# lucidrains/DALLE-pytorch

Hardware: AMD Instinct MI355X
Metric: img-tokens/sec (higher is better)
Workload: dtype bf16; 1 GPU; model=dalle-dim1024-depth12-heads16, reversible=True, global_batch=64, seq_len=1280, image_seq_len=1024, parallelism=dp1, mode=train, eager=False

## Files before the change

### dalle_pytorch_amd/models/reversible.py

```python

import torch
import torch.nn as nn
from torch.autograd.function import Function
from torch.utils.checkpoint import get_device_states, set_device_states


def route_args(router, args, depth):
    routed = [({}, {}) for _ in range(depth)]
    for key, per_layer in router.items():
        if key not in args:
            continue
        val = args[key]
        for i, (f_on, g_on) in enumerate(per_layer):
            if f_on:
                routed[i][0][key] = val
            if g_on:
                routed[i][1][key] = val
    return routed


class Deterministic(nn.Module):

    def __init__(self, net):
        super().__init__()
        self.net = net
        self._cpu_state = None
        self._gpu_devices = None
        self._gpu_states = None
        self._had_gpu = False
        self._autocast = None

    def record_rng(self, *tensors):
        self._cpu_state = torch.get_rng_state()
        if torch.cuda._initialized:
            self._had_gpu = True
            self._gpu_devices, self._gpu_states = get_device_states(*tensors)
        self._autocast = (torch.is_autocast_enabled('cuda'),
                          torch.get_autocast_dtype('cuda'))

    def forward(self, *args, record_rng=False, set_rng=False, **kwargs):
        if record_rng:
            self.record_rng(*args)
        if not set_rng:
            return self.net(*args, **kwargs)
        devices = self._gpu_devices if self._had_gpu else []
        with torch.random.fork_rng(devices=devices, enabled=True):
            torch.set_rng_state(self._cpu_state)
            if self._had_gpu:
                set_device_states(self._gpu_devices, self._gpu_states)
            if self._autocast is not None and self._autocast[0] and torch.cuda.is_available():
                with torch.autocast('cuda', dtype=self._autocast[1], enabled=True):
                    return self.net(*args, **kwargs)
            return self.net(*args, **kwargs)


def _residual_branch(det, inp, residual, record_rng, args):
    if getattr(det.net, 'supports_residual', False):
        return det(inp, residual=residual, record_rng=record_rng, **args)
    return residual + det(inp, record_rng=record_rng, **args)


class ReversibleBlock(nn.Module):

    def __init__(self, f, g):
        super().__init__()
        self.f = Deterministic(f)
        self.g = Deterministic(g)

    def forward(self, x1, x2, f_args={}, g_args={}):
        rec = self.training
        with torch.no_grad():
            y1 = _residual_branch(self.f, x2, x1, rec, f_args)
            y2 = _residual_branch(self.g, y1, x2, rec, g_args)
        return y1, y2

    @staticmethod
    def _replay_grad(det, inp, upstream, args):
        leaf = inp.detach().requires_grad_(True)
        with torch.enable_grad():
            out = det(leaf, set_rng=True, **args)
        torch.autograd.backward(out, upstream)
        return out.detach(), leaf.grad

    def backward_pass(self, y1, y2, dy1, dy2, f_args={}, g_args={}):
        gy1, dy1_via_g = self._replay_grad(self.g, y1, dy2, g_args)
        x2 = y2 - gy1
        dx1 = dy1 + dy1_via_g
        del y2, gy1, dy1, dy1_via_g
        fx2, dx2_via_f = self._replay_grad(self.f, x2, dx1, f_args)
        x1 = y1 - fx2
        dx2 = dy2 + dx2_via_f
        del y1, fx2, dy2, dx2_via_f
        return x1, x2, dx1, dx2


class _ReversibleFunction(Function):
    @staticmethod
    def forward(ctx, x1, x2, blocks, args):
        ctx.args = args
        for block, kw in zip(blocks, args):
            x1, x2 = block(x1, x2, **kw)
        ctx.y1 = x1.detach()
        ctx.y2 = x2.detach()
        ctx.blocks = blocks
        return x1, x2

    @staticmethod
    def backward(ctx, dy1, dy2):
        y1, y2 = ctx.y1, ctx.y2
        for block, kw in zip(ctx.blocks[::-1], ctx.args[::-1]):
            y1, y2, dy1, dy2 = block.backward_pass(y1, y2, dy1, dy2, **kw)
        return dy1, dy2, None, None


class SequentialSequence(nn.Module):
# ... 31 lines not shown
```

### dalle_pytorch_amd/models/transformer.py

```python

from collections import deque
from collections.abc import Iterable
from functools import partial
from itertools import islice, cycle

import torch
import torch.nn.functional as F
from torch import nn

from dalle_pytorch_amd.models.reversible import ReversibleSequence, SequentialSequence
from dalle_pytorch_amd.models.attention import (
    Attention, SparseAttention, SparseConvCausalAttention, SparseAxialCausalAttention)
from dalle_pytorch_amd.models.positional import build_dalle_rotary_table
from dalle_pytorch_amd.ops import geglu
from dalle_pytorch_amd.ops.fp8 import fp8_linear
from dalle_pytorch_amd.ops.fused import (token_shift, token_shift_supported,
                                          layer_norm, add_scaled)


def _as_tuple(val, depth=1):
    return val if isinstance(val, Iterable) else (val,) * depth


class DivideMax(nn.Module):

    def __init__(self, dim):
        super().__init__()
        self.dim = dim

    def forward(self, x):
        maxes = x.amax(dim=self.dim, keepdim=True).detach()
        return x / maxes


class NonCached(nn.Module):

    def __init__(self, fn):
        super().__init__()
        self.fn = fn

# ... 26 lines not shown

    def __init__(self, dim, depth, fn):
        super().__init__()
        init_eps = next(eps for bound, eps in self.INIT_BY_DEPTH
                        if depth <= bound)
        self.scale = nn.Parameter(torch.full((1, 1, dim), init_eps))
        self.fn = fn

    def forward(self, x, residual=None, **kwargs):
        out = self.fn(x, **kwargs)
        if residual is not None:
            return add_scaled(residual, out, self.scale)
        return out * self.scale.to(out.dtype)


class PreNorm(nn.Module):

    def __init__(self, dim, fn, sandwich=False):
        super().__init__()
        self.norm = nn.LayerNorm(dim)
        self.norm_out = nn.LayerNorm(dim) if sandwich else nn.Identity()
        self.fn = fn

    def forward(self, x, **kwargs):
        y = layer_norm(x, self.norm.weight, self.norm.bias, self.norm.eps)
        y = self.fn(y, **kwargs)
        if isinstance(self.norm_out, nn.LayerNorm):
            y = layer_norm(y, self.norm_out.weight, self.norm_out.bias,
                           self.norm_out.eps)
        return y


class GEGLU(nn.Module):
    def forward(self, x):
        return geglu(x)


class FeedForward(nn.Module):

    def __init__(self, dim, dropout=0., mult=4.):
        super().__init__()
        self.net = nn.Sequential(
            nn.Linear(dim, int(dim * mult * 2)),
            GEGLU(),
            nn.Dropout(dropout),
            nn.Linear(int(dim * mult), dim),
        )

    def forward(self, x, cache=None, cache_key=None):
        x = fp8_linear(self.net[0], x)
        x = self.net[2](self.net[1](x))
        return fp8_linear(self.net[3], x)


class PreShiftToken(nn.Module):

    def __init__(self, fn, image_size, seq_len):
        super().__init__()
        self.fn = fn
        self.image_size = image_size
        self.seq_len = seq_len
        self.img_seq_len = image_size ** 2
        self.text_len = seq_len - self.img_seq_len + 1

    def _shift_full(self, x):
        b, n, c = x.shape
        t, S, q = self.text_len, self.image_size, x.shape[-1] // 4
        prev = x[:, :t - 1, :c // 2]
        text = torch.cat((
            torch.cat((x.new_zeros(b, 1, c // 2), prev), dim=1),
            x[:, :t, c // 2:]), dim=-1)
        img = x[:, t:]
        ni = img.shape[1]
        if ni == 0:
# ... 174 lines not shown
```

### dalle_pytorch_amd/ops/fp8.py

```python

import os
import weakref

import torch
import torch.nn.functional as F

from dalle_pytorch_amd.ops.dispatch import hip_module, using_eager_fallback

_FORCED = None
FP8_MAX = 448.0


def set_fp8_enabled(flag):
    global _FORCED
    _FORCED = bool(flag) if flag is not None else None


def fp8_enabled():
    if _FORCED is not None:
        return _FORCED
    return os.environ.get('DALLE_AMD_FP8', '0') == '1'


_w_cache = {}
_generation = 0


def _owner(w):
    base = w._base
    return base if base is not None else w
# ... 121 lines not shown
    return n * 2 >= k * 3


def _fast_dgrad_ok(x, w):
    if using_eager_fallback(x) or x.dtype != torch.bfloat16:
        return False
    rows = x.numel() // x.shape[-1]
    return (rows >= 1024 and rows % 16 == 0 and w.shape[0] % 16 == 0
            and w.shape[1] % 16 == 0 and torch.is_grad_enabled())


def fp8_linear(linear_module, x):
    w = linear_module.weight
    if _fp8_ok(x, w):
        bias = linear_module.bias
        if bias is not None and bias.dtype != torch.bfloat16:
            bias = bias.to(torch.bfloat16)
        return _Fp8LinearFn.apply(x.contiguous(), w, bias)
    if _fast_dgrad_ok(x, w):
        return _FastDgradLinearFn.apply(x.contiguous(), w, linear_module.bias)
    return linear_module(x)


def fp8_linear_raw(x, weight, bias):
    if _fp8_ok(x, weight) and weight.is_contiguous():
        if bias is not None and bias.dtype != torch.bfloat16:
            bias = bias.to(torch.bfloat16)
        return _Fp8LinearFn.apply(x.contiguous(), weight, bias)
    if _fast_dgrad_ok(x, weight) and weight.is_contiguous():
        return _FastDgradLinearFn.apply(x.contiguous(), weight, bias)
    return F.linear(x, weight, bias)
```

### dalle_pytorch_amd/ops/fused.py

```python

import torch
import torch.nn.functional as F

from dalle_pytorch_amd.ops.dispatch import hip_module, using_eager_fallback


class _GegluFn(torch.autograd.Function):
    @staticmethod
    def forward(ctx, x):
        ext = hip_module()
        x = x.contiguous()
        out = ext.geglu_fwd(x)
        ctx.save_for_backward(x)
        return out

    @staticmethod
    def backward(ctx, dout):
        ext = hip_module()
        (x,) = ctx.saved_tensors
        return ext.geglu_bwd(x, dout.contiguous())


def geglu(x: torch.Tensor) -> torch.Tensor:
    if using_eager_fallback(x) or x.shape[-1] % 16:
# ... 35 lines not shown
        out = ext.resls_fwd(x.contiguous(), y, gf)
        ctx.save_for_backward(y, gf)
        ctx.gamma_meta = (gamma.shape, gamma.dtype)
        return out

    @staticmethod
    def backward(ctx, dout):
        ext = hip_module()
        y, gf = ctx.saved_tensors
        dout = dout.contiguous()
        dy, dgamma = ext.resls_bwd(dout, y, gf)
        shape, dtype = ctx.gamma_meta
        return dout, dy, dgamma.reshape(shape).to(dtype)


def add_scaled(x, y, gamma):
    if (x.is_cuda and x.dtype == torch.bfloat16 and y.dtype == torch.bfloat16
            and not using_eager_fallback(x) and x.shape[-1] % 8 == 0
            and x.shape[-1] // 8 <= 256 and 256 % (x.shape[-1] // 8) == 0):
        return _AddScaledFn.apply(x, y, gamma)
    return x + y * gamma.to(y.dtype)


class _LayerNormFn(torch.autograd.Function):
    @staticmethod
    def forward(ctx, x, weight, bias, eps):
        ext = hip_module()
        y, mean, rstd = ext.ln_fwd(x.contiguous(), weight, bias, eps)
        ctx.save_for_backward(x, weight, mean, rstd)
        return y

    @staticmethod
    def backward(ctx, dy):
        ext = hip_module()
        x, weight, mean, rstd = ctx.saved_tensors
        dx, dgamma, dbeta = ext.ln_bwd(x, dy.contiguous(), weight, mean, rstd)
        return dx, dgamma.to(weight.dtype), dbeta.to(weight.dtype), None


_LN_DIMS = (512, 1024, 1536, 2048)


def layer_norm(x, weight, bias, eps=1e-5):
    if (x.is_cuda and x.dtype == torch.bfloat16 and x.shape[-1] in _LN_DIMS
            and not using_eager_fallback(x)):
        return _LayerNormFn.apply(x, weight, bias, eps)
    if weight is not None and weight.dtype != x.dtype and x.dtype != torch.float32:
        weight = weight.to(x.dtype)
        bias = bias.to(x.dtype) if bias is not None else None
    return F.layer_norm(x, (x.shape[-1],), weight, bias, eps)
```

### dalle_pytorch_amd/ops/hip/hip_ops.hip

```cpp

#include <torch/extension.h>
#include <ATen/hip/HIPContext.h>
#include <hip/hip_runtime.h>

#define DEVFN __device__ __forceinline__

using bf16x8 = __attribute__((ext_vector_type(8))) short;
using bf16x4 = __attribute__((ext_vector_type(4))) short;
using f32x4 = __attribute__((ext_vector_type(4))) float;
using int4v = __attribute__((ext_vector_type(4))) int;

constexpr float NEG_INF = -INFINITY;

DEVFN float bf2f(short u) {
  union { unsigned int i; float f; } c;
  c.i = (unsigned int)(unsigned short)u << 16;
  return c.f;
}
DEVFN short f2bf(float f) {
  union { unsigned int i; float f; } c;
  c.f = f;
  unsigned int r = c.i + 0x7fff + ((c.i >> 16) & 1);
  return (short)(r >> 16);
}
// ... 1621 lines not shown
  #pragma unroll
  for (int e = 0; e < 8; ++e) g[e] = gamma[ch + e];
  for (long r = (long)blockIdx.x * rpp + rg; r < rows;
       r += (long)gridDim.x * rpp) {
    const long base = r * dim + ch;
    int4v dv = *reinterpret_cast<const int4v*>(dout + base);
    int4v yv = *reinterpret_cast<const int4v*>(y + base);
    const short* ds_ = reinterpret_cast<const short*>(&dv);
    const short* ys = reinterpret_cast<const short*>(&yv);
    short o[8];
    #pragma unroll
    for (int e = 0; e < 8; ++e) {
      const float d = bf2f(ds_[e]);
      o[e] = f2bf(g[e] * d);
      dg[e] += d * bf2f(ys[e]);
    }
    *reinterpret_cast<int4v*>(dy + base) = *reinterpret_cast<int4v*>(o);
  }
  const long prow = (long)blockIdx.x * rpp + rg;
  #pragma unroll
  for (int e = 0; e < 8; ++e) dg_part[prow * dim + ch + e] = dg[e];
}


template <int CPT>
__global__ __launch_bounds__(256)
void dec_prelude_kernel(
    const short* __restrict__ x,
    const short* __restrict__ y,
    const float* __restrict__ scale,
    const float* __restrict__ w,
    const float* __restrict__ bia,
    short* __restrict__ xn,
    short* __restrict__ z,
    short* __restrict__ ring,
    const long* __restrict__ offset,
    long rows, float eps, int S, int text_len) {
  constexpr int dim = CPT * 256;
  __shared__ float stat[8];
  const long row = blockIdx.x;
  const int tid = threadIdx.x;
  const int c0 = tid * CPT;
  const short* xr = x + row * (long)dim;
  const short* yr = y ? y + row * (long)dim : nullptr;

  float sum = 0.f, sq = 0.f;
// ... 241 lines not shown
                                      long rows, int H) {
  const long row = blockIdx.y;
  const int i0 = (blockIdx.x * blockDim.x + threadIdx.x) * 8;
  if (row >= rows || i0 >= H) return;
  int4v av = *reinterpret_cast<const int4v*>(x + row * (2L * H) + i0);
  int4v gv = *reinterpret_cast<const int4v*>(x + row * (2L * H) + H + i0);
  int4v dv = *reinterpret_cast<const int4v*>(dout + row * (long)H + i0);
  const short* a = reinterpret_cast<const short*>(&av);
  const short* g = reinterpret_cast<const short*>(&gv);
  const short* d = reinterpret_cast<const short*>(&dv);
  short da[8], dg[8];
  #pragma unroll
  for (int e = 0; e < 8; ++e) {
    const float afv = bf2f(a[e]), gfv = bf2f(g[e]), dfv = bf2f(d[e]);
    da[e] = f2bf(dfv * gelu_f(gfv));
    dg[e] = f2bf(dfv * afv * gelu_grad_f(gfv));
  }
  *reinterpret_cast<int4v*>(dx + row * (2L * H) + i0) =
      *reinterpret_cast<const int4v*>(da);
  *reinterpret_cast<int4v*>(dx + row * (2L * H) + H + i0) =
      *reinterpret_cast<const int4v*>(dg);
}

template <typename T>
__global__ void geglu_fwd_kernel(const T* __restrict__ x, T* __restrict__ out,
                                 long rows, int H) {
  const long row = blockIdx.y;
  const int i0 = (blockIdx.x * blockDim.x + threadIdx.x) * 8;
  if (row >= rows || i0 >= H) return;
  const T* a = x + row * (2L * H) + i0;
  const T* g = a + H;
  T* o = out + row * (long)H + i0;
  #pragma unroll
  for (int e = 0; e < 8; ++e)
    if (i0 + e < H) o[e] = T(float(a[e]) * gelu_f(float(g[e])));
}

template <typename T>
__global__ void geglu_bwd_kernel(const T* __restrict__ x,
                                 const T* __restrict__ dout,
                                 T* __restrict__ dx, long rows, int H) {
  const long row = blockIdx.y;
  const int i0 = (blockIdx.x * blockDim.x + threadIdx.x) * 8;
  if (row >= rows || i0 >= H) return;
  const T* a = x + row * (2L * H) + i0;
  const T* g = a + H;
// ... 473 lines not shown
  const int i = blockIdx.x * blockDim.x + threadIdx.x;
  if (i >= dim) return;
  const long g0 = *offset - text_len;
  const long g = g0 < 0 ? 0 : g0;
  const int pos = (int)(g % S);
  const int prev = (int)(((g - 1) % S + S) % S);
  const int half = dim / 2, quarter = dim / 4;

  short val;
  if (i < quarter) {
    val = ring[((long)bi * S + pos) * half + i];
  } else if (i < half) {
    val = (g % S == 0) ? (short)0
        : ring[((long)bi * S + prev) * half + i];
  } else {
    val = x[(long)bi * dim + i];
  }
  if (i < half) ring[((long)bi * S + pos) * half + i] = x[(long)bi * dim + i];
  out[(long)bi * dim + i] = val;
}



template <int PER>
__global__ __launch_bounds__(256)
void ln_fwd_kernel(const short* __restrict__ x, const float* __restrict__ w,
                   const float* __restrict__ bia, short* __restrict__ y,
                   float* __restrict__ mean_out, float* __restrict__ rstd_out,
                   long rows, float eps) {
  constexpr int per = PER;
  constexpr int dim = PER * 64;
  const long row0 = ((long)blockIdx.x * 4 + (threadIdx.x >> 6)) * 2;
  const int lane = threadIdx.x & 63;
  if (row0 >= rows) return;
  const bool two = row0 + 1 < rows;

  float vals[2][PER];
  #pragma unroll
  for (int rr = 0; rr < 2; ++rr) {
    if (rr && !two) break;
    const short* xr = x + (row0 + rr) * (long)dim;
    #pragma unroll
    for (int i = 0; i < per; i += 8) {
      int4v v = *reinterpret_cast<const int4v*>(xr + lane * per + i);
      const short* vs = reinterpret_cast<const short*>(&v);
      #pragma unroll
      for (int e = 0; e < 8; ++e) vals[rr][i + e] = bf2f(vs[e]);
    }
  }
  #pragma unroll
  for (int rr = 0; rr < 2; ++rr) {
    if (rr && !two) break;
    float sum = 0.f, sq = 0.f;
    #pragma unroll
    for (int i = 0; i < per; ++i) {
      sum += vals[rr][i];
      sq += vals[rr][i] * vals[rr][i];
    }
    #pragma unroll
    for (int sft = 32; sft > 0; sft >>= 1) {
      sum += __shfl_xor(sum, sft);
      sq += __shfl_xor(sq, sft);
    }
    const float mu = sum / dim;
    const float var = sq / dim - mu * mu;
    const float rstd = __frsqrt_rn(var + eps);
    if (lane == 0) {
      mean_out[row0 + rr] = mu;
      rstd_out[row0 + rr] = rstd;
    }
    short* yr = y + (row0 + rr) * (long)dim;
    #pragma unroll
    for (int i = 0; i < per; i += 8) {
      short out8[8];
      #pragma unroll
      for (int e = 0; e < 8; ++e) {
        const int d = lane * per + i + e;
        out8[e] = f2bf((vals[rr][i + e] - mu) * rstd * w[d] + bia[d]);
      }
      *reinterpret_cast<int4v*>(yr + lane * per + i) =
          *reinterpret_cast<const int4v*>(out8);
    }
  }
}

template <int PER>
__global__ __launch_bounds__(256)
void ln_bwd_kernel(const short* __restrict__ x, const short* __restrict__ dy,
                   const float* __restrict__ w,
                   const float* __restrict__ mean_in,
                   const float* __restrict__ rstd_in,
                   short* __restrict__ dx,
                   float* __restrict__ dgamma_part,
                   float* __restrict__ dbeta_part,
                   long rows) {
  constexpr int per = PER;
  constexpr int dim = PER * 64;
  const int block_row0 = blockIdx.x * 4;
  const int wrow = threadIdx.x >> 6;
  const int lane = threadIdx.x & 63;
  const int gridrows = gridDim.x * 4;

  float dgp[PER], dbp[PER];
  #pragma unroll
  for (int i = 0; i < per; ++i) { dgp[i] = 0.f; dbp[i] = 0.f; }

  for (long row = block_row0 + wrow; row < rows; row += gridrows) {
    const short* xr = x + row * dim;
    const short* dyr = dy + row * dim;
    const float mu = mean_in[row];
    const float rstd = rstd_in[row];

    float xh[PER], g[PER];
    float s1 = 0.f, s2 = 0.f;
    #pragma unroll
    for (int i = 0; i < per; i += 8) {
      int4v xv = *reinterpret_cast<const int4v*>(xr + lane * per + i);
      int4v dv = *reinterpret_cast<const int4v*>(dyr + lane * per + i);
      const short* xs = reinterpret_cast<const short*>(&xv);
      const short* ds_ = reinterpret_cast<const short*>(&dv);
      #pragma unroll
      for (int e = 0; e < 8; ++e) {
        const int d = lane * per + i + e;
        const float xhat = (bf2f(xs[e]) - mu) * rstd;
        const float dyv = bf2f(ds_[e]);
        const float gv = dyv * w[d];
        xh[i + e] = xhat;
        g[i + e] = gv;
        s1 += gv;
        s2 += gv * xhat;
        dgp[i + e] += dyv * xhat;
        dbp[i + e] += dyv;
      }
    }
    #pragma unroll
    for (int sft = 32; sft > 0; sft >>= 1) {
      s1 += __shfl_xor(s1, sft);
      s2 += __shfl_xor(s2, sft);
    }
    s1 /= dim;
    s2 /= dim;
    short* dxr = dx + row * (long)dim;
    #pragma unroll
    for (int i = 0; i < per; i += 8) {
      short out8[8];
      #pragma unroll
      for (int e = 0; e < 8; ++e)
        out8[e] = f2bf((g[i + e] - s1 - xh[i + e] * s2) * rstd);
      *reinterpret_cast<int4v*>(dxr + lane * per + i) =
          *reinterpret_cast<const int4v*>(out8);
    }
  }
  float* dgr = dgamma_part + ((long)blockIdx.x * 4 + wrow) * dim;
  float* dbr = dbeta_part + ((long)blockIdx.x * 4 + wrow) * dim;
  #pragma unroll
  for (int i = 0; i < per; ++i) {
    dgr[lane * per + i] = dgp[i];
    dbr[lane * per + i] = dbp[i];
  }
}


__global__ void mfma_probe_kernel(const short* __restrict__ A,
                                  const short* __restrict__ B,
                                  float* __restrict__ C) {
  const int lane = threadIdx.x & 63;
  const int lq = lane & 15, grp = lane >> 4;
  bf16x8 af = *reinterpret_cast<const bf16x8*>(A + lq * 32 + 8 * grp);
  bf16x8 bf;
  #pragma unroll
  for (int e = 0; e < 8; ++e) bf[e] = B[(8 * grp + e) * 16 + lq];
// ... 246 lines not shown
  return out;
}

torch::Tensor geglu_bwd(torch::Tensor x, torch::Tensor dout) {
  CHK(x.is_cuda() && x.is_contiguous() && dout.is_contiguous());
  const int H = (int)x.size(-1) / 2;
  const long rows = x.numel() / (2L * H);
  auto dx = torch::empty_like(x);
  dim3 grid((H + 256 * 8 - 1) / (256 * 8), rows);
  if (x.dtype() == torch::kBFloat16 && H % 8 == 0) {
    hipLaunchKernelGGL(geglu_bwd_bf16_kernel, grid, dim3(256), 0, cur_stream(),
                       reinterpret_cast<const short*>(x.data_ptr()),
                       reinterpret_cast<const short*>(dout.data_ptr()),
                       reinterpret_cast<short*>(dx.data_ptr()), rows, H);
    return dx;
  }
  AT_DISPATCH_FLOATING_TYPES_AND2(at::ScalarType::BFloat16, at::ScalarType::Half,
                                  x.scalar_type(), "geglu_bwd", [&] {
    hipLaunchKernelGGL(geglu_bwd_kernel<scalar_t>, grid, dim3(256), 0, cur_stream(),
                       x.data_ptr<scalar_t>(), dout.data_ptr<scalar_t>(),
                       dx.data_ptr<scalar_t>(), rows, H);
  });
  return dx;
}

torch::Tensor fa_decode(torch::Tensor qkv, torch::Tensor kc, torch::Tensor vc,
                        std::optional<torch::Tensor> cosv,
                        std::optional<torch::Tensor> sinv,
                        torch::Tensor offset,
                        std::optional<torch::Tensor> pattern,
                        double scale,
                        std::optional<torch::Tensor> live,
                        std::optional<torch::Tensor> live_cnt) {
  CHK(qkv.is_cuda() && qkv.dtype() == torch::kBFloat16 && qkv.is_contiguous());
  CHK(kc.is_contiguous() && vc.is_contiguous());
  const int b = kc.size(0), h = kc.size(1), N = kc.size(2);
  CHK(kc.size(3) == 64 && N <= DEC_MAXN);
  CHK(offset.dtype() == torch::kLong);
  int rot = 0;
  const float* cp = nullptr;
  const float* sp = nullptr;
  if (cosv.has_value()) {
    rot = cosv->size(1);
    cp = cosv->data_ptr<float>();
    sp = sinv->data_ptr<float>();
  }
// ... 105 lines not shown
                     C.data_ptr<float>());
  return C;
}


std::vector<torch::Tensor> ln_fwd(torch::Tensor x, torch::Tensor w,
                                  torch::Tensor b, double eps) {
  CHK(x.is_cuda() && x.dtype() == torch::kBFloat16 && x.is_contiguous());
  const int dim = x.size(-1);

  const long rows = x.numel() / dim;
  auto y = torch::empty_like(x);
  auto mean = torch::empty({rows}, x.options().dtype(torch::kFloat32));
  auto rstd = torch::empty_like(mean);
  auto wf = w.to(torch::kFloat32).contiguous();
  auto bf_ = b.to(torch::kFloat32).contiguous();
  dim3 grid((rows + 7) / 8);
  auto launch = [&](auto kern) {
    hipLaunchKernelGGL(kern, grid, dim3(256), 0, cur_stream(),
                       reinterpret_cast<const short*>(x.data_ptr()),
                       wf.data_ptr<float>(), bf_.data_ptr<float>(),
                       reinterpret_cast<short*>(y.data_ptr()),
                       mean.data_ptr<float>(), rstd.data_ptr<float>(),
                       rows, (float)eps);
  };
  switch (dim) {
    case 512: launch(ln_fwd_kernel<8>); break;
    case 1024: launch(ln_fwd_kernel<16>); break;
    case 1536: launch(ln_fwd_kernel<24>); break;
    case 2048: launch(ln_fwd_kernel<32>); break;
    default: TORCH_CHECK(false, "ln_fwd: unsupported dim ", dim);
  }
  return {y, mean, rstd};
}

std::vector<torch::Tensor> ln_bwd(torch::Tensor x, torch::Tensor dy,
                                  torch::Tensor w, torch::Tensor mean,
                                  torch::Tensor rstd) {
  CHK(x.is_cuda() && x.is_contiguous() && dy.is_contiguous());
  const int dim = x.size(-1);
  const long rows = x.numel() / dim;
  auto dx = torch::empty_like(x);
  const long cap = std::min<long>((rows + 3) / 4, 512);
  auto dgp = torch::empty({cap * 4, (long)dim}, x.options().dtype(torch::kFloat32));
  auto dbp = torch::empty_like(dgp);
  auto wf = w.to(torch::kFloat32).contiguous();
  dim3 grid(cap);
  auto launch = [&](auto kern) {
    hipLaunchKernelGGL(kern, grid, dim3(256), 0, cur_stream(),
                       reinterpret_cast<const short*>(x.data_ptr()),
                       reinterpret_cast<const short*>(dy.data_ptr()),
                       wf.data_ptr<float>(), mean.data_ptr<float>(),
                       rstd.data_ptr<float>(),
                       reinterpret_cast<short*>(dx.data_ptr()),
                       dgp.data_ptr<float>(), dbp.data_ptr<float>(), rows);
  };
  switch (dim) {
    case 512: launch(ln_bwd_kernel<8>); break;
    case 1024: launch(ln_bwd_kernel<16>); break;
    case 1536: launch(ln_bwd_kernel<24>); break;
    case 2048: launch(ln_bwd_kernel<32>); break;
    default: TORCH_CHECK(false, "ln_bwd: unsupported dim ", dim);
  }
  auto dgamma = dgp.sum(0);
  auto dbeta = dbp.sum(0);
  return {dx, dgamma, dbeta};
}

std::vector<torch::Tensor> dec_prelude(
    torch::Tensor x, std::optional<torch::Tensor> y,
    std::optional<torch::Tensor> scale,
    torch::Tensor w, torch::Tensor b,
    std::optional<torch::Tensor> ring, torch::Tensor offset,
    double eps, int64_t S, int64_t text_len) {
  CHK(x.is_cuda() && x.dtype() == torch::kBFloat16 && x.is_contiguous());
  CHK(w.dtype() == torch::kFloat32 && b.dtype() == torch::kFloat32);
  const int dim = x.size(-1);
  const long rows = x.numel() / dim;
  const short* yp = nullptr;
  const float* sp_ = nullptr;
  torch::Tensor xn = x;
  if (y.has_value()) {
    CHK(y->is_contiguous() && scale.has_value());
    CHK(scale->dtype() == torch::kFloat32 && scale->is_contiguous());
    yp = reinterpret_cast<const short*>(y->data_ptr());
    sp_ = scale->data_ptr<float>();
    xn = torch::empty_like(x);
  }
  short* rp = nullptr;
// ... 194 lines not shown
                     gamma.data_ptr<float>(),
                     reinterpret_cast<short*>(out.data_ptr()), rows, dim);
  return out;
}

std::vector<torch::Tensor> resls_bwd(torch::Tensor dout, torch::Tensor y,
                                     torch::Tensor gamma) {
  CHK(dout.is_cuda() && dout.dtype() == torch::kBFloat16);
  CHK(dout.is_contiguous() && y.is_contiguous() && gamma.is_contiguous());
  const int dim = dout.size(-1);
  const long rows = dout.numel() / dim;
  auto dy = torch::empty_like(dout);
  const int rpp = 256 / (dim >> 3);
  const long nb = std::min<long>((rows + rpp - 1) / rpp, 1024);
  auto dgp = torch::zeros({nb * rpp, (long)dim},
                          dout.options().dtype(torch::kFloat32));
  hipLaunchKernelGGL(resls_bwd_kernel, dim3(nb), dim3(256), 0, cur_stream(),
                     reinterpret_cast<const short*>(dout.data_ptr()),
                     reinterpret_cast<const short*>(y.data_ptr()),
                     gamma.data_ptr<float>(),
                     reinterpret_cast<short*>(dy.data_ptr()),
                     dgp.data_ptr<float>(), rows, dim);
  return {dy, dgp.sum(0)};
}

PYBIND11_MODULE(TORCH_EXTENSION_NAME, m) {
  m.def("resls_fwd", &resls_fwd, "fused residual + per-channel scale fwd");
  m.def("resls_bwd", &resls_bwd, "fused residual + per-channel scale bwd");
  m.def("quant_fp8", &quant_fp8, "bf16 -> e4m3 one-pass quantize");
  m.def("sample_topk_gumbel", &sample_topk_gumbel,
        py::arg("logits"), py::arg("noise"), py::arg("k"),
        py::arg("temperature"), py::arg("out_tok") = std::nullopt,
        py::arg("seq") = std::nullopt, py::arg("seq_ptr") = std::nullopt,
        "fused top-k threshold + gumbel argmax sampling");
  m.def("amax_bf16", &amax_bf16, "abs-max of a bf16 tensor (one pass)");
  m.def("sk2", &sk2,
        py::arg("x"), py::arg("wp"), py::arg("bias"), py::arg("N"),
        py::arg("K"), py::arg("mode"), py::arg("wscale") = 1.0,
        "decode skinny GEMM on packed bf16/e4m3 weights "
        "(fused bias/geglu/fp32 head)");
  m.def("skinny_gemm", &skinny_gemm,
        "skinny-M weights-streaming GEMM (decode projections)",
        py::arg("x"), py::arg("w"), py::arg("bias") = std::nullopt);
  m.def("dec_prelude", &dec_prelude,
        "fused decode residual + LayerNorm + token-shift");
  m.def("permlane_probe", &permlane_probe,
        "v_permlane32_swap_b32 semantics probe");
  m.def("fa_fwd", &fa_fwd, "flash attention forward (gfx950, d=64)",
        py::arg("q"), py::arg("k"), py::arg("v"), py::arg("scale"),
        py::arg("causal"), py::arg("key_mask"), py::arg("static_mask"),
        py::arg("tile_map"), py::arg("out_bnhd"),
        py::arg("ax_t") = 0, py::arg("ax_S") = 0, py::arg("ax_axis") = -1);
  m.def("fa_bwd", &fa_bwd, "flash attention backward (gfx950, d=64)",
        py::arg("q"), py::arg("k"), py::arg("v"), py::arg("out"),
        py::arg("lse"), py::arg("dout"), py::arg("scale"), py::arg("causal"),
        py::arg("key_mask"), py::arg("static_mask"), py::arg("tile_map"),
        py::arg("tile_map_t"), py::arg("out_bnhd"),
        py::arg("grad_lse") = std::nullopt,
        py::arg("ax_t") = 0, py::arg("ax_S") = 0, py::arg("ax_axis") = -1);
  m.def("rope_split_fwd", &rope_split_fwd,
        "fused qkv split + rotary (q,k,v all rotated)");
  m.def("rope_split_bwd", &rope_split_bwd, "rope_split backward");
  m.def("token_shift", &token_shift, "fused token shift (fwd/transpose)");
  m.def("fa_decode", &fa_decode, "fused single-token decode attention");
  m.def("shift_decode", &shift_decode, "fused single-token token shift");
  m.def("ln_fwd", &ln_fwd, "fused LayerNorm forward (bf16 rows)");
  m.def("ln_bwd", &ln_bwd, "fused LayerNorm backward");
  m.def("geglu_fwd", &geglu_fwd, "fused GEGLU forward");
  m.def("geglu_bwd", &geglu_bwd, "fused GEGLU backward");
  m.def("mfma_probe", &mfma_probe, "MFMA 16x16x32 bf16 layout probe");
}
```

Baseline: 294,900 img_tokens_per_sec.

## Fuse reversible replay tail, LayerNorm+token shift, residual-grad fold, and linear+GEGLU bias grad

Several fusions land together. A rev_replay kernel computes the reconstructed input, the scaled upstream gradient and the per-channel gamma gradient in one pass, and the residual stream gradient is folded into the LayerNorm backward through dres. LayerNorm is fused with token shift in both forward and backward. The FF first linear is paired with GEGLU in a custom autograd function whose backward emits the bias gradient as a column sum. The aim is fewer elementwise kernel launches and memory passes in the backward replay, in exchange for more custom kernels and more complex autograd plumbing.

```diff
diff --git a/dalle_pytorch_amd/models/reversible.py b/dalle_pytorch_amd/models/reversible.py
--- a/dalle_pytorch_amd/models/reversible.py
+++ b/dalle_pytorch_amd/models/reversible.py
@@ -3,6 +3,8 @@
 import torch.nn as nn
 from torch.autograd.function import Function
 from torch.utils.checkpoint import get_device_states, set_device_states
+
+from dalle_pytorch_amd.ops.fused import fusion_enabled, rev_replay
 
 
 def route_args(router, args, depth):
@@ -38,11 +40,13 @@
         self._autocast = (torch.is_autocast_enabled('cuda'),
                           torch.get_autocast_dtype('cuda'))
 
-    def forward(self, *args, record_rng=False, set_rng=False, **kwargs):
+    def forward(self, *args, record_rng=False, set_rng=False, inner=False,
+                **kwargs):
         if record_rng:
             self.record_rng(*args)
+        net = self.net.fn if inner else self.net
         if not set_rng:
-            return self.net(*args, **kwargs)
+            return net(*args, **kwargs)
         devices = self._gpu_devices if self._had_gpu else []
         with torch.random.fork_rng(devices=devices, enabled=True):
             torch.set_rng_state(self._cpu_state)
@@ -50,8 +54,8 @@
                 set_device_states(self._gpu_devices, self._gpu_states)
             if self._autocast is not None and self._autocast[0] and torch.cuda.is_available():
                 with torch.autocast('cuda', dtype=self._autocast[1], enabled=True):
-                    return self.net(*args, **kwargs)
-            return self.net(*args, **kwargs)
+                    return net(*args, **kwargs)
+            return net(*args, **kwargs)
 
 
 def _residual_branch(det, inp, residual, record_rng, args):
@@ -82,15 +86,39 @@
         torch.autograd.backward(out, upstream)
         return out.detach(), leaf.grad
 
+    @staticmethod
+    def _replay_fused(det, inp, out, upstream, stream_grad, args):
+        ls = det.net
+        fn = ls.fn
+        leaf = inp.detach().requires_grad_(True)
+        folds = getattr(fn, 'fuses_dres', None)
+        fold = (folds is not None and folds(leaf)
+                and stream_grad.dtype == leaf.dtype
+                and stream_grad.shape == leaf.shape)
+        if fold:
+            args = dict(args, dres=stream_grad)
+        with torch.enable_grad():
+            o = det(leaf, set_rng=True, inner=True, **args)
+        rec, d_o, dscale = rev_replay(o, ls.scale, out, upstream)
+        if ls.scale.requires_grad:
+            torch.autograd.backward([o, ls.scale], [d_o, dscale])
+        else:
+            torch.autograd.backward(o, d_o)
+        return rec, (leaf.grad if fold else stream_grad + leaf.grad)
+
+    def _invert(self, det, inp, out, upstream, stream_grad, args):
+        if (getattr(det.net, 'supports_residual', False)
+                and fusion_enabled('REV_REPLAY')):
+            return self._replay_fused(det, inp, out, upstream, stream_grad,
+                                      args)
+        b_out, via = self._replay_grad(det, inp, upstream, args)
+        return out - b_out, stream_grad + via
+
     def backward_pass(self, y1, y2, dy1, dy2, f_args={}, g_args={}):
-        gy1, dy1_via_g = self._replay_grad(self.g, y1, dy2, g_args)
-        x2 = y2 - gy1
-        dx1 = dy1 + dy1_via_g
-        del y2, gy1, dy1, dy1_via_g
-        fx2, dx2_via_f = self._replay_grad(self.f, x2, dx1, f_args)
-        x1 = y1 - fx2
-        dx2 = dy2 + dx2_via_f
-        del y1, fx2, dy2, dx2_via_f
+        x2, dx1 = self._invert(self.g, y1, y2, dy2, dy1, g_args)
+        del y2, dy1
+        x1, dx2 = self._invert(self.f, x2, y1, dx1, dy2, f_args)
+        del y1, dy2
         return x1, x2, dx1, dx2
 
 
diff --git a/dalle_pytorch_amd/models/transformer.py b/dalle_pytorch_amd/models/transformer.py
--- a/dalle_pytorch_amd/models/transformer.py
+++ b/dalle_pytorch_amd/models/transformer.py
@@ -13,9 +13,11 @@
     Attention, SparseAttention, SparseConvCausalAttention, SparseAxialCausalAttention)
 from dalle_pytorch_amd.models.positional import build_dalle_rotary_table
 from dalle_pytorch_amd.ops import geglu
-from dalle_pytorch_amd.ops.fp8 import fp8_linear
+from dalle_pytorch_amd.ops.fp8 import fp8_linear, linear_geglu, linear_geglu_ok
 from dalle_pytorch_amd.ops.fused import (token_shift, token_shift_supported,
-                                          layer_norm, add_scaled)
+                                          layer_norm, layer_norm_fused,
+                                          ln_shift, ln_shift_supported,
+                                          add_scaled)
 
 
 def _as_tuple(val, depth=1):
@@ -88,9 +90,29 @@
         self.norm_out = nn.LayerNorm(dim) if sandwich else nn.Identity()
         self.fn = fn
 
-    def forward(self, x, **kwargs):
-        y = layer_norm(x, self.norm.weight, self.norm.bias, self.norm.eps)
-        y = self.fn(y, **kwargs)
+    def fuses_dres(self, x):
+        return layer_norm_fused(x)
+
+    def _shift_child(self, x, kwargs):
+        wrap = self.fn
+        shift = wrap.fn if isinstance(wrap, CachedAs) else None
+        if (isinstance(shift, PreShiftToken) and kwargs.get('cache') is None
+                and x.dim() == 3 and x.shape[1] >= shift.text_len
+                and ln_shift_supported(x)):
+            return shift
+        return None
+
+    def forward(self, x, dres=None, **kwargs):
+        shift = self._shift_child(x, kwargs)
+        if shift is not None:
+            y = ln_shift(x, self.norm.weight, self.norm.bias, self.norm.eps,
+                         shift.text_len, shift.image_size, dres)
+            inner = {k: v for k, v in kwargs.items() if k != 'cache'}
+            y = shift.fn(y, **inner)
+        else:
+            y = layer_norm(x, self.norm.weight, self.norm.bias, self.norm.eps,
+                           dres)
+            y = self.fn(y, **kwargs)
         if isinstance(self.norm_out, nn.LayerNorm):
             y = layer_norm(y, self.norm_out.weight, self.norm_out.bias,
                            self.norm_out.eps)
@@ -114,8 +136,11 @@
         )
 
     def forward(self, x, cache=None, cache_key=None):
-        x = fp8_linear(self.net[0], x)
-        x = self.net[2](self.net[1](x))
+        if linear_geglu_ok(self.net[0], x):
+            x = linear_geglu(self.net[0], x)
+        else:
+            x = self.net[1](fp8_linear(self.net[0], x))
+        x = self.net[2](x)
         return fp8_linear(self.net[3], x)
 
 
diff --git a/dalle_pytorch_amd/ops/fp8.py b/dalle_pytorch_amd/ops/fp8.py
--- a/dalle_pytorch_amd/ops/fp8.py
+++ b/dalle_pytorch_amd/ops/fp8.py
@@ -6,6 +6,7 @@
 import torch.nn.functional as F
 
 from dalle_pytorch_amd.ops.dispatch import hip_module, using_eager_fallback
+from dalle_pytorch_amd.ops.fused import fusion_enabled, geglu_bwd_colsum
 
 _FORCED = None
 FP8_MAX = 448.0
@@ -173,6 +174,51 @@
     return linear_module(x)
 
 
+class _LinearGegluFn(torch.autograd.Function):
+
+    @staticmethod
+    def forward(ctx, x, weight, bias):
+        ext = hip_module()
+        bb = bias if bias.dtype == torch.bfloat16 else bias.to(torch.bfloat16)
+        x2 = x.reshape(-1, x.shape[-1])
+        if _fp8_ok(x, weight):
+            xq, xs = _quant(x2, ext)
+            wq, ws = _quant_weight(weight, ext)
+            h = torch._scaled_mm(xq, wq.t(), scale_a=xs, scale_b=ws,
+                                 bias=bb, out_dtype=torch.bfloat16)
+        else:
+            h = F.linear(x, _cached_bf16(weight), bb)
+        h = h.reshape(-1, weight.shape[0])
+        out = ext.geglu_fwd(h)
+        ctx.save_for_backward(x2, weight, h)
+        ctx.bias_dtype = bias.dtype
+        return out.reshape(*x.shape[:-1], weight.shape[0] // 2)
+
+    @staticmethod
+    def backward(ctx, dout):
+        x2, weight, h = ctx.saved_tensors
+        do2 = dout.reshape(-1, dout.shape[-1]).contiguous()
+        dh, db = geglu_bwd_colsum(h, do2)
+        wt = _transposed_weight(weight)
+        dx = (dh @ wt.t()).reshape(*dout.shape[:-1], weight.shape[1])
+        dw = dh.t() @ x2.to(dh.dtype)
+        return dx, dw.to(weight.dtype), db.to(ctx.bias_dtype)
+
+
+def linear_geglu_ok(linear_module, x):
+    w = linear_module.weight
+    n_out = w.shape[0]
+    h8 = n_out // 16
+    return (fusion_enabled('FF1_BIAS') and linear_module.bias is not None
+            and (_fp8_ok(x, w) or _fast_dgrad_ok(x, w))
+            and n_out % 16 == 0 and (h8 % 256 == 0 or 256 % h8 == 0))
+
+
+def linear_geglu(linear_module, x):
+    return _LinearGegluFn.apply(x.contiguous(), linear_module.weight,
+                                linear_module.bias)
+
+
 def fp8_linear_raw(x, weight, bias):
     if _fp8_ok(x, weight) and weight.is_contiguous():
         if bias is not None and bias.dtype != torch.bfloat16:
diff --git a/dalle_pytorch_amd/ops/fused.py b/dalle_pytorch_amd/ops/fused.py
--- a/dalle_pytorch_amd/ops/fused.py
+++ b/dalle_pytorch_amd/ops/fused.py
@@ -1,3 +1,5 @@
+
+import os
 
 import torch
 import torch.nn.functional as F
@@ -81,30 +83,152 @@
     return x + y * gamma.to(y.dtype)
 
 
+def fusion_enabled(name):
+    return os.environ.get('DALLE_AMD_' + name, '1') == '1'
+
+
 class _LayerNormFn(torch.autograd.Function):
-    @staticmethod
-    def forward(ctx, x, weight, bias, eps):
-        ext = hip_module()
-        y, mean, rstd = ext.ln_fwd(x.contiguous(), weight, bias, eps)
+
+    @staticmethod
+    def forward(ctx, x, weight, bias, eps, dres=None):
+        ext = hip_module()
+        x = x.contiguous()
+        y, mean, rstd = ext.ln_fwd(x, weight, bias, eps)
         ctx.save_for_backward(x, weight, mean, rstd)
+        ctx.dres = dres
         return y
 
     @staticmethod
     def backward(ctx, dy):
         ext = hip_module()
         x, weight, mean, rstd = ctx.saved_tensors
-        dx, dgamma, dbeta = ext.ln_bwd(x, dy.contiguous(), weight, mean, rstd)
-        return dx, dgamma.to(weight.dtype), dbeta.to(weight.dtype), None
+        dres, ctx.dres = ctx.dres, None
+        if dres is None:
+            dx, dgamma, dbeta = ext.ln_bwd(x, dy.contiguous(), weight, mean,
+                                           rstd)
+        else:
+            dx, dgamma, dbeta = ext.ln_shift_bwd(
+                x, dy.contiguous(), weight, mean, rstd, dres.contiguous())
+        return dx, dgamma.to(weight.dtype), dbeta.to(weight.dtype), None, None
+
+
+class _LnShiftFn(torch.autograd.Function):
+
+    @staticmethod
+    def forward(ctx, x, weight, bias, eps, text_len, image_size, dres=None):
+        ext = hip_module()
+        x = x.contiguous()
+        y, mean, rstd = ext.ln_shift_fwd(x, weight, bias, eps, text_len,
+                                         image_size)
+        ctx.save_for_backward(x, weight, mean, rstd)
+        ctx.shift = (text_len, image_size)
+        ctx.dres = dres
+        return y
+
+    @staticmethod
+    def backward(ctx, dy):
+        ext = hip_module()
+        x, weight, mean, rstd = ctx.saved_tensors
+        dres, ctx.dres = ctx.dres, None
+        dx, dgamma, dbeta = ext.ln_shift_bwd(
+            x, dy.contiguous(), weight, mean, rstd,
+            None if dres is None else dres.contiguous(), *ctx.shift)
+        return (dx, dgamma.to(weight.dtype), dbeta.to(weight.dtype),
+                None, None, None, None)
 
 
 _LN_DIMS = (512, 1024, 1536, 2048)
 
 
-def layer_norm(x, weight, bias, eps=1e-5):
-    if (x.is_cuda and x.dtype == torch.bfloat16 and x.shape[-1] in _LN_DIMS
-            and not using_eager_fallback(x)):
-        return _LayerNormFn.apply(x, weight, bias, eps)
+def layer_norm_fused(x):
+    return (x.is_cuda and x.dtype == torch.bfloat16 and x.shape[-1] in _LN_DIMS
+            and not using_eager_fallback(x))
+
+
+def layer_norm(x, weight, bias, eps=1e-5, dres=None):
+    if layer_norm_fused(x):
+        return _LayerNormFn.apply(x, weight, bias, eps, dres)
+    assert dres is None, 'dres needs the fused LayerNorm path'
     if weight is not None and weight.dtype != x.dtype and x.dtype != torch.float32:
         weight = weight.to(x.dtype)
         bias = bias.to(x.dtype) if bias is not None else None
     return F.layer_norm(x, (x.shape[-1],), weight, bias, eps)
+
+
+def ln_shift_supported(x):
+    return (fusion_enabled('LN_SHIFT') and x.dim() == 3 and layer_norm_fused(x)
+            and token_shift_supported(x))
+
+
+def ln_shift(x, weight, bias, eps, text_len, image_size, dres=None):
+    if ln_shift_supported(x):
+        return _LnShiftFn.apply(x, weight, bias, eps, text_len, image_size,
+                                dres)
+    y = layer_norm(x, weight, bias, eps, dres)
+    if token_shift_supported(y):
+        return token_shift(y, text_len, image_size)
+    return _shift_full_eager(y, text_len, image_size)
+
+
+def _shift_full_eager(x, t, S):
+    b, n, c = x.shape
+    q = c // 4
+    prev = x[:, :t - 1, :c // 2]
+    text = torch.cat((
+        torch.cat((x.new_zeros(b, 1, c // 2), prev), dim=1),
+        x[:, :t, c // 2:]), dim=-1)
+    img = x[:, t:]
+    ni = img.shape[1]
+    if ni == 0:
+        return text
+    g = F.pad(img, (0, 0, 0, S * S - ni)).view(b, S, S, c)
+    top = torch.cat((g.new_zeros(b, 1, S, q), g[:, :-1, :, :q]), dim=1)
+    left = torch.cat((g.new_zeros(b, S, 1, q), g[:, :, :-1, q:2 * q]), dim=2)
+    img = torch.cat((top, left, g[..., 2 * q:]), dim=-1)
+    return torch.cat((text, img.view(b, S * S, c)[:, :ni]), dim=1)
+
+
+def rev_replay_supported(o, y, d):
+    return (o.is_cuda and o.dtype == torch.bfloat16
+            and y.dtype == torch.bfloat16 and d.dtype == torch.bfloat16
+            and o.shape == y.shape == d.shape
+            and not using_eager_fallback(o) and o.shape[-1] % 8 == 0
+            and o.shape[-1] // 8 <= 256 and 256 % (o.shape[-1] // 8) == 0)
+
+
+def rev_replay(o, gamma, y, d):
+    o, y, d = o.detach(), y.detach(), d.detach()
+    if rev_replay_supported(o, y, d):
+        ext = hip_module()
+        gf = gamma.detach().reshape(-1).float().contiguous()
+        x_rec, d_o, dg = ext.rev_replay(o.contiguous(), gf, y.contiguous(),
+                                        d.contiguous())
+        return x_rec, d_o, dg.reshape(gamma.shape).to(gamma.dtype)
+    g = gamma.detach()
+    x_rec = (y - g * o).to(y.dtype)
+    d_o = (g * d).to(o.dtype)
+    dg = (d.float() * o.float()).reshape(-1, o.shape[-1]).sum(0)
+    return x_rec, d_o, dg.reshape(gamma.shape).to(gamma.dtype)
+
+
+def geglu_bwd_colsum_supported(x):
+    h8 = x.shape[-1] // 16
+    return (x.is_cuda and x.dtype == torch.bfloat16 and x.shape[-1] % 16 == 0
+            and h8 > 0 and not using_eager_fallback(x)
+            and (h8 % 256 == 0 or 256 % h8 == 0))
+
+
+def geglu_bwd_colsum(x, dout):
+    if geglu_bwd_colsum_supported(x) and dout.dtype == torch.bfloat16:
+        ext = hip_module()
+        dx, cs = ext.geglu_bwd_colsum(x.contiguous(), dout.contiguous())
+        return dx, cs
+    if not using_eager_fallback(x):
+        dx = hip_module().geglu_bwd(x.contiguous(), dout.contiguous())
+    else:
+        with torch.enable_grad():
+            xl = x.detach().requires_grad_(True)
+            a, b = xl.chunk(2, dim=-1)
+            out = a * F.gelu(b)
+        dx, = torch.autograd.grad(out, xl, dout)
+    return dx, dx.reshape(-1, dx.shape[-1]).float().sum(0)
diff --git a/dalle_pytorch_amd/ops/hip/hip_ops.hip b/dalle_pytorch_amd/ops/hip/hip_ops.hip
--- a/dalle_pytorch_amd/ops/hip/hip_ops.hip
+++ b/dalle_pytorch_amd/ops/hip/hip_ops.hip
@@ -1667,6 +1667,45 @@
   for (int e = 0; e < 8; ++e) dg_part[prow * dim + ch + e] = dg[e];
 }
 
+__global__ __launch_bounds__(256)
+void rev_replay_kernel(const short* __restrict__ o, const short* __restrict__ y,
+                       const short* __restrict__ d,
+                       const float* __restrict__ gamma,
+                       short* __restrict__ xrec, short* __restrict__ dout,
+                       float* __restrict__ dg_part,
+                       long rows, int dim) {
+  const int cpr = dim >> 3;
+  const int rpp = 256 / cpr;
+  const int rg = threadIdx.x / cpr;
+  const int ch = (threadIdx.x % cpr) * 8;
+  float g[8], dg[8] = {0, 0, 0, 0, 0, 0, 0, 0};
+  #pragma unroll
+  for (int e = 0; e < 8; ++e) g[e] = gamma[ch + e];
+  for (long r = (long)blockIdx.x * rpp + rg; r < rows;
+       r += (long)gridDim.x * rpp) {
+    const long base = r * dim + ch;
+    int4v ov = *reinterpret_cast<const int4v*>(o + base);
+    int4v yv = *reinterpret_cast<const int4v*>(y + base);
+    int4v dv = *reinterpret_cast<const int4v*>(d + base);
+    const short* os = reinterpret_cast<const short*>(&ov);
+    const short* ys = reinterpret_cast<const short*>(&yv);
+    const short* ds_ = reinterpret_cast<const short*>(&dv);
+    short xo[8], go[8];
+    #pragma unroll
+    for (int e = 0; e < 8; ++e) {
+      const float of = bf2f(os[e]), df = bf2f(ds_[e]);
+      xo[e] = f2bf(bf2f(ys[e]) - g[e] * of);
+      go[e] = f2bf(g[e] * df);
+      dg[e] += df * of;
+    }
+    *reinterpret_cast<int4v*>(xrec + base) = *reinterpret_cast<int4v*>(xo);
+    *reinterpret_cast<int4v*>(dout + base) = *reinterpret_cast<int4v*>(go);
+  }
+  const long prow = (long)blockIdx.x * rpp + rg;
+  #pragma unroll
+  for (int e = 0; e < 8; ++e) dg_part[prow * dim + ch + e] = dg[e];
+}
+
 
 template <int CPT>
 __global__ __launch_bounds__(256)
@@ -1954,6 +1993,51 @@
       *reinterpret_cast<const int4v*>(dg);
 }
 
+__global__ __launch_bounds__(256)
+void geglu_bwd_colsum_kernel(const short* __restrict__ x,
+                             const short* __restrict__ dout,
+                             short* __restrict__ dx,
+                             float* __restrict__ part,
+                             long rows, int H) {
+  const int cpr = H >> 3;
+  const int tpr = cpr < 256 ? cpr : 256;
+  const int rpp = 256 / tpr;
+  const int rg = threadIdx.x / tpr;
+  const int i0 = (blockIdx.x * tpr + threadIdx.x % tpr) * 8;
+  const long rstride = (long)gridDim.y * rpp;
+  float sa[8], sg[8];
+  #pragma unroll
+  for (int e = 0; e < 8; ++e) { sa[e] = 0.f; sg[e] = 0.f; }
+
+  for (long row = (long)blockIdx.y * rpp + rg; row < rows; row += rstride) {
+    int4v av = *reinterpret_cast<const int4v*>(x + row * (2L * H) + i0);
+    int4v gv = *reinterpret_cast<const int4v*>(x + row * (2L * H) + H + i0);
+    int4v dv = *reinterpret_cast<const int4v*>(dout + row * (long)H + i0);
+    const short* a = reinterpret_cast<const short*>(&av);
+    const short* g = reinterpret_cast<const short*>(&gv);
+    const short* d = reinterpret_cast<const short*>(&dv);
+    short da[8], dg[8];
+    #pragma unroll
+    for (int e = 0; e < 8; ++e) {
+      const float afv = bf2f(a[e]), gfv = bf2f(g[e]), dfv = bf2f(d[e]);
+      da[e] = f2bf(dfv * gelu_f(gfv));
+      dg[e] = f2bf(dfv * afv * gelu_grad_f(gfv));
+      sa[e] += bf2f(da[e]);
+      sg[e] += bf2f(dg[e]);
+    }
+    *reinterpret_cast<int4v*>(dx + row * (2L * H) + i0) =
+        *reinterpret_cast<const int4v*>(da);
+    *reinterpret_cast<int4v*>(dx + row * (2L * H) + H + i0) =
+        *reinterpret_cast<const int4v*>(dg);
+  }
+  float* pr = part + ((long)blockIdx.y * rpp + rg) * (2L * H);
+  #pragma unroll
+  for (int e = 0; e < 8; ++e) {
+    pr[i0 + e] = sa[e];
+    pr[H + i0 + e] = sg[e];
+  }
+}
+
 template <typename T>
 __global__ void geglu_fwd_kernel(const T* __restrict__ x, T* __restrict__ out,
                                  long rows, int H) {
@@ -2473,12 +2557,13 @@
 
 
 
-template <int PER>
+template <int PER, bool SHIFT = false>
 __global__ __launch_bounds__(256)
+__attribute__((amdgpu_waves_per_eu(SHIFT && PER == 16 ? 6 : 1)))
 void ln_fwd_kernel(const short* __restrict__ x, const float* __restrict__ w,
                    const float* __restrict__ bia, short* __restrict__ y,
                    float* __restrict__ mean_out, float* __restrict__ rstd_out,
-                   long rows, float eps) {
+                   long rows, float eps, int n, int text_len, int S) {
   constexpr int per = PER;
   constexpr int dim = PER * 64;
   const long row0 = ((long)blockIdx.x * 4 + (threadIdx.x >> 6)) * 2;
@@ -2521,6 +2606,39 @@
       rstd_out[row0 + rr] = rstd;
     }
     short* yr = y + (row0 + rr) * (long)dim;
+    bool keep = true;
+    bool zfill = false;
+    unsigned loff = lane * per;
+    if constexpr (SHIFT) {
+      const int region = lane >> 4;
+      if (region < 2) {
+        const int pos = (int)((unsigned)__builtin_amdgcn_readfirstlane(
+            (int)(row0 + rr)) % (unsigned)n);
+        int dst = 1;
+        if (pos < text_len) {
+          keep = pos + 1 < text_len;
+          zfill = pos == 0;
+        } else {
+          const int g = pos - text_len;
+          const int gr = g / S, gc = g - gr * S;
+          if (region == 0) {
+            keep = pos + S < n;
+            dst = S;
+            zfill = gr == 0;
+          } else {
+            keep = gc + 1 < S && pos + 1 < n;
+            zfill = gc == 0;
+          }
+        }
+        if (zfill) {
+          #pragma unroll
+          for (int i = 0; i < per; i += 8)
+            *reinterpret_cast<int4v*>(yr + lane * per + i) = int4v{0, 0, 0, 0};
+        }
+        loff += (unsigned)(dst * dim);
+      }
+    }
+    if (!keep) continue;
     #pragma unroll
     for (int i = 0; i < per; i += 8) {
       short out8[8];
@@ -2529,13 +2647,13 @@
         const int d = lane * per + i + e;
         out8[e] = f2bf((vals[rr][i + e] - mu) * rstd * w[d] + bia[d]);
       }
-      *reinterpret_cast<int4v*>(yr + lane * per + i) =
+      *reinterpret_cast<int4v*>(yr + loff + i) =
           *reinterpret_cast<const int4v*>(out8);
     }
   }
 }
 
-template <int PER>
+template <int PER, bool SHIFT = false, bool DRES = false>
 __global__ __launch_bounds__(256)
 void ln_bwd_kernel(const short* __restrict__ x, const short* __restrict__ dy,
                    const float* __restrict__ w,
@@ -2544,7 +2662,8 @@
                    short* __restrict__ dx,
                    float* __restrict__ dgamma_part,
                    float* __restrict__ dbeta_part,
-                   long rows) {
+                   long rows, const short* __restrict__ dres,
+                   int n, int text_len, int S) {
   constexpr int per = PER;
   constexpr int dim = PER * 64;
   const int block_row0 = blockIdx.x * 4;
@@ -2561,13 +2680,23 @@
     const short* dyr = dy + row * dim;
     const float mu = mean_in[row];
     const float rstd = rstd_in[row];
+    bool dyzero = false;
+    if constexpr (SHIFT) {
+      const int pos = (int)((unsigned)row % (unsigned)n);
+      int srcpos;
+      token_shift_src(pos, lane * per * 2, n, text_len, S, dim, dim / 2, 1,
+                      &srcpos, &dyzero);
+      dyr += (long)(srcpos - pos) * dim;
+    }
 
     float xh[PER], g[PER];
     float s1 = 0.f, s2 = 0.f;
     #pragma unroll
     for (int i = 0; i < per; i += 8) {
       int4v xv = *reinterpret_cast<const int4v*>(xr + lane * per + i);
-      int4v dv = *reinterpret_cast<const int4v*>(dyr + lane * per + i);
+      int4v dv = int4v{0, 0, 0, 0};
+      if (!SHIFT || !dyzero)
+        dv = *reinterpret_cast<const int4v*>(dyr + lane * per + i);
       const short* xs = reinterpret_cast<const short*>(&xv);
       const short* ds_ = reinterpret_cast<const short*>(&dv);
       #pragma unroll
@@ -2595,9 +2724,19 @@
     #pragma unroll
     for (int i = 0; i < per; i += 8) {
       short out8[8];
-      #pragma unroll
-      for (int e = 0; e < 8; ++e)
-        out8[e] = f2bf((g[i + e] - s1 - xh[i + e] * s2) * rstd);
+      if constexpr (DRES) {
+        int4v rv = *reinterpret_cast<const int4v*>(
+            dres + row * (long)dim + lane * per + i);
+        const short* rs = reinterpret_cast<const short*>(&rv);
+        #pragma unroll
+        for (int e = 0; e < 8; ++e)
+          out8[e] = f2bf(bf2f(rs[e]) +
+                         (g[i + e] - s1 - xh[i + e] * s2) * rstd);
+      } else {
+        #pragma unroll
+        for (int e = 0; e < 8; ++e)
+          out8[e] = f2bf((g[i + e] - s1 - xh[i + e] * s2) * rstd);
+      }
       *reinterpret_cast<int4v*>(dxr + lane * per + i) =
           *reinterpret_cast<const int4v*>(out8);
     }
@@ -2890,6 +3029,43 @@
                        dx.data_ptr<scalar_t>(), rows, H);
   });
   return dx;
+}
+
+std::vector<torch::Tensor> geglu_bwd_colsum(torch::Tensor x, torch::Tensor dout) {
+  CHK(x.is_cuda() && x.is_contiguous() && dout.is_contiguous());
+  CHK(x.dtype() == torch::kBFloat16 && dout.dtype() == torch::kBFloat16);
+  const int H = (int)x.size(-1) / 2;
+  CHK(H > 0 && H % 8 == 0 && x.size(-1) == 2L * H && dout.size(-1) == H);
+  const int cpr = H / 8;
+  CHK(cpr % 256 == 0 || 256 % cpr == 0);
+  const long rows = x.numel() / (2L * H);
+  CHK(dout.numel() == rows * (long)H);
+  auto dx = torch::empty_like(x);
+  const int tpr = cpr < 256 ? cpr : 256;
+  const int rpp = 256 / tpr;
+  const int nbx = cpr / tpr;
+  static const long resident = [] {
+    int per_cu = 0, dev = 0;
+    hipDeviceProp_t prop;
+    if (hipOccupancyMaxActiveBlocksPerMultiprocessor(
+            &per_cu, geglu_bwd_colsum_kernel, 256, 0) != hipSuccess ||
+        hipGetDevice(&dev) != hipSuccess ||
+        hipGetDeviceProperties(&prop, dev) != hipSuccess || per_cu < 1)
+      return 1024L;
+    return (long)per_cu * prop.multiProcessorCount;
+  }();
+  const long want = std::max<long>(resident / nbx, 1);
+  const long nby = std::max<long>(
+      std::min<long>((rows + rpp - 1) / rpp, want), 1);
+  auto part = torch::empty({nby * rpp, 2L * H},
+                           x.options().dtype(torch::kFloat32));
+  hipLaunchKernelGGL(geglu_bwd_colsum_kernel, dim3(nbx, nby), dim3(256), 0,
+                     cur_stream(),
+                     reinterpret_cast<const short*>(x.data_ptr()),
+                     reinterpret_cast<const short*>(dout.data_ptr()),
+                     reinterpret_cast<short*>(dx.data_ptr()),
+                     part.data_ptr<float>(), rows, H);
+  return {dx, part.sum(0)};
 }
 
 torch::Tensor fa_decode(torch::Tensor qkv, torch::Tensor kc, torch::Tensor vc,
@@ -3041,7 +3217,7 @@
                        wf.data_ptr<float>(), bf_.data_ptr<float>(),
                        reinterpret_cast<short*>(y.data_ptr()),
                        mean.data_ptr<float>(), rstd.data_ptr<float>(),
-                       rows, (float)eps);
+                       rows, (float)eps, 0, 0, 1);
   };
   switch (dim) {
     case 512: launch(ln_fwd_kernel<8>); break;
@@ -3072,7 +3248,8 @@
                        wf.data_ptr<float>(), mean.data_ptr<float>(),
                        rstd.data_ptr<float>(),
                        reinterpret_cast<short*>(dx.data_ptr()),
-                       dgp.data_ptr<float>(), dbp.data_ptr<float>(), rows);
+                       dgp.data_ptr<float>(), dbp.data_ptr<float>(), rows,
+                       (const short*)nullptr, 0, 0, 1);
   };
   switch (dim) {
     case 512: launch(ln_bwd_kernel<8>); break;
@@ -3084,6 +3261,97 @@
   auto dgamma = dgp.sum(0);
   auto dbeta = dbp.sum(0);
   return {dx, dgamma, dbeta};
+}
+
+std::vector<torch::Tensor> ln_shift_fwd(torch::Tensor x, torch::Tensor w,
+                                        torch::Tensor b, double eps,
+                                        int64_t text_len, int64_t image_size) {
+  CHK(x.is_cuda() && x.dtype() == torch::kBFloat16 && x.is_contiguous());
+  CHK(x.dim() == 3 && image_size >= 1 && text_len >= 0);
+  const int dim = x.size(-1);
+  const int n = x.size(1);
+  CHK(n >= text_len);
+  const long rows = x.numel() / dim;
+  CHK(rows < (1L << 31));
+  auto y = torch::empty_like(x);
+  auto mean = torch::empty({rows}, x.options().dtype(torch::kFloat32));
+  auto rstd = torch::empty_like(mean);
+  auto wf = w.to(torch::kFloat32).contiguous();
+  auto bf_ = b.to(torch::kFloat32).contiguous();
+  dim3 grid((rows + 7) / 8);
+  auto launch = [&](auto kern) {
+    hipLaunchKernelGGL(kern, grid, dim3(256), 0, cur_stream(),
+                       reinterpret_cast<const short*>(x.data_ptr()),
+                       wf.data_ptr<float>(), bf_.data_ptr<float>(),
+                       reinterpret_cast<short*>(y.data_ptr()),
+                       mean.data_ptr<float>(), rstd.data_ptr<float>(),
+                       rows, (float)eps, n, (int)text_len, (int)image_size);
+  };
+  switch (dim) {
+    case 512: launch(ln_fwd_kernel<8, true>); break;
+    case 1024: launch(ln_fwd_kernel<16, true>); break;
+    case 1536: launch(ln_fwd_kernel<24, true>); break;
+    case 2048: launch(ln_fwd_kernel<32, true>); break;
+    default: TORCH_CHECK(false, "ln_shift_fwd: unsupported dim ", dim);
+  }
+  return {y, mean, rstd};
+}
+
+std::vector<torch::Tensor> ln_shift_bwd(torch::Tensor x, torch::Tensor dy,
+                                        torch::Tensor w, torch::Tensor mean,
+                                        torch::Tensor rstd,
+                                        std::optional<torch::Tensor> dres,
+                                        int64_t text_len, int64_t image_size) {
+  CHK(x.is_cuda() && x.dtype() == torch::kBFloat16 && x.is_contiguous());
+  CHK(dy.is_contiguous() && dy.dtype() == torch::kBFloat16 &&
+      dy.numel() == x.numel());
+  const bool shift = image_size > 0;
+  const bool has_res = dres.has_value();
+  CHK(shift || has_res);
+  const int dim = x.size(-1);
+  const long rows = x.numel() / dim;
+  CHK(mean.numel() == rows && rstd.numel() == rows);
+  int n = 0;
+  if (shift) {
+    CHK(x.dim() == 3 && text_len >= 0 && x.size(1) >= text_len);
+    CHK(rows < (1L << 31));
+    n = x.size(1);
+  }
+  const short* rp = nullptr;
+  if (has_res) {
+    CHK(dres->is_cuda() && dres->is_contiguous() &&
+        dres->dtype() == torch::kBFloat16 && dres->numel() == x.numel());
+    rp = reinterpret_cast<const short*>(dres->data_ptr());
+  }
+  auto dx = torch::empty_like(x);
+  const long cap = std::min<long>((rows + 3) / 4, 512);
+  auto dgp = torch::empty({cap * 4, (long)dim}, x.options().dtype(torch::kFloat32));
+  auto dbp = torch::empty_like(dgp);
+  auto wf = w.to(torch::kFloat32).contiguous();
+  dim3 grid(cap);
+  auto launch = [&](auto kern) {
+    hipLaunchKernelGGL(kern, grid, dim3(256), 0, cur_stream(),
+                       reinterpret_cast<const short*>(x.data_ptr()),
+                       reinterpret_cast<const short*>(dy.data_ptr()),
+                       wf.data_ptr<float>(), mean.data_ptr<float>(),
+                       rstd.data_ptr<float>(),
+                       reinterpret_cast<short*>(dx.data_ptr()),
+                       dgp.data_ptr<float>(), dbp.data_ptr<float>(), rows,
+                       rp, n, (int)text_len, (int)image_size);
+  };
+  #define LN_SB(PER)                                                    \
+    if (shift && has_res) launch(ln_bwd_kernel<PER, true, true>);       \
+    else if (shift)       launch(ln_bwd_kernel<PER, true, false>);      \
+    else                  launch(ln_bwd_kernel<PER, false, true>);
+  switch (dim) {
+    case 512: LN_SB(8); break;
+    case 1024: LN_SB(16); break;
+    case 1536: LN_SB(24); break;
+    case 2048: LN_SB(32); break;
+    default: TORCH_CHECK(false, "ln_shift_bwd: unsupported dim ", dim);
+  }
+  #undef LN_SB
+  return {dx, dgp.sum(0), dbp.sum(0)};
 }
 
 std::vector<torch::Tensor> dec_prelude(
@@ -3324,6 +3592,35 @@
                      reinterpret_cast<short*>(dy.data_ptr()),
                      dgp.data_ptr<float>(), rows, dim);
   return {dy, dgp.sum(0)};
+}
+
+std::vector<torch::Tensor> rev_replay(torch::Tensor o, torch::Tensor gamma,
+                                      torch::Tensor y, torch::Tensor d) {
+  CHK(o.is_cuda() && o.dtype() == torch::kBFloat16 &&
+      y.dtype() == torch::kBFloat16 && d.dtype() == torch::kBFloat16);
+  CHK(o.is_contiguous() && y.is_contiguous() && d.is_contiguous() &&
+      gamma.is_contiguous());
+  CHK(gamma.dtype() == torch::kFloat32);
+  const int dim = o.size(-1);
+  CHK(dim == gamma.numel() && (dim & 7) == 0 && (dim >> 3) <= 256 &&
+      (256 % (dim >> 3)) == 0);
+  CHK(y.numel() == o.numel() && d.numel() == o.numel());
+  const long rows = o.numel() / dim;
+  auto xrec = torch::empty_like(o);
+  auto dout = torch::empty_like(o);
+  const int rpp = 256 / (dim >> 3);
+  const long nb = std::max<long>(std::min<long>((rows + rpp - 1) / rpp, 1024), 1);
+  auto dgp = torch::empty({nb * rpp, (long)dim},
+                          o.options().dtype(torch::kFloat32));
+  hipLaunchKernelGGL(rev_replay_kernel, dim3(nb), dim3(256), 0, cur_stream(),
+                     reinterpret_cast<const short*>(o.data_ptr()),
+                     reinterpret_cast<const short*>(y.data_ptr()),
+                     reinterpret_cast<const short*>(d.data_ptr()),
+                     gamma.data_ptr<float>(),
+                     reinterpret_cast<short*>(xrec.data_ptr()),
+                     reinterpret_cast<short*>(dout.data_ptr()),
+                     dgp.data_ptr<float>(), rows, dim);
+  return {xrec, dout, dgp.sum(0)};
 }
 
 PYBIND11_MODULE(TORCH_EXTENSION_NAME, m) {
@@ -3370,5 +3667,15 @@
   m.def("ln_bwd", &ln_bwd, "fused LayerNorm backward");
   m.def("geglu_fwd", &geglu_fwd, "fused GEGLU forward");
   m.def("geglu_bwd", &geglu_bwd, "fused GEGLU backward");
+  m.def("geglu_bwd_colsum", &geglu_bwd_colsum,
+        "fused GEGLU backward + fp32 column sums of dx");
+  m.def("ln_shift_fwd", &ln_shift_fwd, "LayerNorm + token shift forward");
+  m.def("ln_shift_bwd", &ln_shift_bwd,
+        "LayerNorm backward with shifted dy and/or residual gradient",
+        py::arg("x"), py::arg("dy"), py::arg("w"), py::arg("mean"),
+        py::arg("rstd"), py::arg("dres") = py::none(),
+        py::arg("text_len") = 0, py::arg("image_size") = 0);
+  m.def("rev_replay", &rev_replay,
+        "reversible replay tail: x_rec, d_o, dgamma in one pass");
   m.def("mfma_probe", &mfma_probe, "MFMA 16x16x32 bf16 layout probe");
 }
```

After: 309,700 img_tokens_per_sec (median of 6 runs). +5.0%, better.
